# dusanerdeljan/stereo-depth

Measured on AMD Instinct MI355X. Metric: disparity maps/sec (stereo pairs/sec) at 1242x375 D=128, higher is better.
Workload: dtype f32

## Files before the change

stereo-depth_amd/csrc/k_match_fast.h:

```cpp
#pragma once
#include "smx_common.h"

namespace smx {

constexpr int FA_HALO = 11;
constexpr int FA_VALID = 64 - 2 * FA_HALO;
#ifndef SMX_FA_WAVES
#define SMX_FA_WAVES 4
#endif
constexpr int FA_WAVES = SMX_FA_WAVES;
#ifndef SMX_FA_DS_WAVES
#define SMX_FA_DS_WAVES 8
#endif
constexpr int FA_DS_WAVES = SMX_FA_DS_WAVES;
#ifndef SMX_FA_TH
#define SMX_FA_TH 24
#endif
constexpr int FA_TH = SMX_FA_TH;
#ifndef SMX_FA_TH_SMALL
#define SMX_FA_TH_SMALL 8
#endif
constexpr int FA_TH_SMALL = SMX_FA_TH_SMALL;
constexpr int FA_TH_SMALL_TALL = 12;
constexpr int FA_TH_SMALL_MID = 10;
#ifndef SMX_FA_PF
#define SMX_FA_PF 2
#endif
constexpr int FA_PF = SMX_FA_PF;
#ifndef SMX_FA_SB_PERIOD
#define SMX_FA_SB_PERIOD 2
#endif
#ifndef SMX_FA_OCC
#define SMX_FA_OCC 3
#endif
#ifndef SMX_FA_DS_OCC
#define SMX_FA_DS_OCC 4
#endif
constexpr int FA_WGCOLS = FA_VALID * FA_WAVES + 2 * FA_HALO;
#ifndef SMX_FA_WIDE_FROM
#define SMX_FA_WIDE_FROM (256 - FA_WGCOLS + 1)
#endif
constexpr int FA_WIDE_FROM = SMX_FA_WIDE_FROM;
constexpr int FA_MID_PITCH = 288;
#ifdef SMX_FA_NO_MID_PITCH
constexpr int FA_MID_UPTO = 0;
#else
constexpr int FA_MID_UPTO = FA_MID_PITCH - FA_WGCOLS + 1;
#endif
constexpr int FA_PL = (FA_VALID * FA_WAVES + 2 * FA_HALO + 7) & ~7;
constexpr int FA_BITWORDS = 64;
__host__ __device__ inline int fast_bitwords(int Dd) {
    return Dd > FA_BITWORDS * 32 ? 2 : ((Dd + 1) & ~1);
}
#define SMX_FOR_EACH_NEEDED(tbl, lo, hi, all_needed, lane, dd, rows, BODY)                                      \
    for (int g_ = (lo); g_ < (hi); g_ += 64) {                                                                  \
        const int idx_ = g_ + (lane);                                                                           \
        unsigned word_ = 0u;                                                                                    \
        if (idx_ < (hi)) word_ = (all_needed) ? ~0u : (tbl)[idx_];                                              \
        unsigned long long m_ = __ballot(word_ != 0u);                                                          \
        while (m_ != 0ull) {                                                                                    \
            const int k_ = __builtin_ctzll(m_);                                                                 \
            m_ &= m_ - 1ull;                                                                                    \
            const int dd = g_ + k_;                                                                             \
            const unsigned rows = (unsigned)__builtin_amdgcn_readlane((int)word_, k_);                          \
            BODY                                                                                                \
        }                                                                                                       \
    }

constexpr int FA_DENSE_MAX_TH = 27;
constexpr int FA_XROW = 64 + 12;
#ifndef SMX_FA_XCH_ROWS
#define SMX_FA_XCH_ROWS 2
#endif
constexpr int FA_XCH_ROWS = SMX_FA_XCH_ROWS;
constexpr int FA_XCH_FLOATS = 2 * FA_XCH_ROWS * FA_XROW;

__host__ __device__ constexpr int fast_merge_rows(int th) { return th > 8 ? (th + 1) / 2 : th; }

__host__ __device__ constexpr bool fast_prefix_exact(int th, int k_max) {
    return (long long)(th + 11) * 48195 * k_max * k_max < (1LL << 24);
}
__host__ __device__ constexpr bool fast_prefix_form(int th, int pr, bool p1only, bool dsplit, int pk16, bool argb, bool dense) {
#ifdef SMX_FA_NO_PREFIX
    return false;
#else
    if (pk16 != 2 || !fast_prefix_exact(th, 2)) return false;
    if (dsplit) return th == FA_TH_SMALL_TALL;
    (void)pr; (void)p1only; (void)argb; (void)dense;
    return true;
#endif
}

template <int PR> inline size_t fast_lds_bytes(int th, int Dd, bool dsplit = false) {
    const size_t nw = dsplit ? FA_DS_WAVES : FA_WAVES;
    return (size_t)(th + 22) * (FA_PL + PR) * sizeof(unsigned short) + nw * fast_bitwords(Dd) * sizeof(unsigned) +
           nw * FA_XCH_FLOATS * sizeof(float) + (dsplit ? nw * fast_merge_rows(th) * 64 * 2 * sizeof(float) : 0);
}

__device__ __forceinline__ float dpp_shr1(float v) {
    return __int_as_float(__builtin_amdgcn_update_dpp(0, __float_as_int(v), 0x138, 0xf, 0xf, true));
}
__device__ __forceinline__ float dpp_shl1(float v) {
    return __int_as_float(__builtin_amdgcn_update_dpp(0, __float_as_int(v), 0x130, 0xf, 0xf, true));
}
__device__ __forceinline__ unsigned dppu_sum3(unsigned v) {
    unsigned t = (unsigned)__builtin_amdgcn_update_dpp(0, (int)v, 0x138, 0xf, 0xf, true) + v;
    asm("" : "+v"(t));
    return t + (unsigned)__builtin_amdgcn_update_dpp(0, (int)v, 0x130, 0xf, 0xf, true);
}

__device__ __forceinline__ void store_u32off(float *base_uniform, unsigned off_elems, float v) {
    *(float *)((char *)base_uniform + (size_t)(off_elems * 4u)) = v;
}

__device__ __forceinline__ void atomic_or_u32off(unsigned *base_uniform, unsigned off_words, unsigned bits) {
    atomicOr((unsigned *)((char *)base_uniform + (size_t)(off_words * 4u)), bits);
}

template <int NK, int NW, bool ROUND = false>
__device__ __forceinline__ void fast_stage(unsigned short *tile, int pitch, const float *img, int h, int w,
                                           int row0, int col0, int rows, int cols, float unit, int wv, int lane) {
    int cidx[NK];
    {
        int c = wrapi(col0 + lane, w);
        const int cstep = 64 % w;
#pragma unroll
        for (int k = 0; k < NK; ++k) {
            cidx[k] = c;
            c += cstep;
            c = c >= w ? c - w : c;
        }
    }
    int ra = wrapi(row0 + wv, h);
    const int rstep = (2 * NW) % h, rhalf = NW % h;
    for (int r = wv; r < rows; r += 2 * NW) {
        const int r2 = r + NW;
        int rb = ra + rhalf;
        rb = rb >= h ? rb - h : rb;
        const float *src = img + (size_t)ra * w;
        const float *src2 = img + (size_t)(r2 < rows ? rb : ra) * w;
        float v[NK], v2[NK];
#pragma unroll
        for (int k = 0; k < NK; ++k) {
            const bool in = lane + 64 * k < cols;
            v[k] = in ? src[cidx[k]] : 0.f;
            v2[k] = in ? src2[cidx[k]] : 0.f;
        }
        unsigned short *dst = tile + r * pitch, *dst2 = tile + r2 * pitch;
#pragma unroll
        for (int k = 0; k < NK; ++k) {
            if (lane + 64 * k < cols) {
                dst[lane + 64 * k] = (unsigned short)(ROUND ? unit * v[k] + 0.5f : unit * v[k]);
                if (r2 < rows) dst2[lane + 64 * k] = (unsigned short)(ROUND ? unit * v2[k] + 0.5f : unit * v2[k]);
            }
        }
        ra += rstep;
        ra = ra >= h ? ra - h : ra;
    }
}

__host__ __device__ constexpr bool fast_units_form(int th, int pr, bool dsplit, bool argb) {
#ifdef SMX_FA_STAGE_F32
    (void)th; (void)pr; (void)dsplit; (void)argb;
    return false;
#else
    return dsplit ? th != FA_TH_SMALL_MID : (pr != 320 || argb);
#endif
}
#ifndef SMX_FA_STAGE_LOADS
#define SMX_FA_STAGE_LOADS 8
#endif
template <int NK, int NW, bool WITH_LEFT>
__device__ __forceinline__ void fast_stage_units(unsigned short *tile, int pitch, const unsigned short *img, int col0, int cols,
                                                 unsigned short *ltile, const unsigned short *limg, int lcol0, int lcols,
                                                 int h, int w, int upitch, int row0, int rows, int wv, int lane) {
    constexpr int NB = SMX_FA_STAGE_LOADS / (NK + (WITH_LEFT ? 1 : 0));
    typedef unsigned u32x2 __attribute__((ext_vector_type(2)));
    unsigned coff[NK], lcoff = 0u;
    bool in[NK], lin = false;
#pragma unroll
    for (int k = 0; k < NK; ++k) {
        in[k] = 256 * k + 4 * lane < cols;
        coff[k] = 2u * (unsigned)wrapi(col0 + 256 * k + 4 * lane, w);
    }
    if (WITH_LEFT) {
        lin = 4 * lane < lcols;
        lcoff = 2u * (unsigned)wrapi(lcol0 + 4 * lane, w);
    }
    const int wvu = __builtin_amdgcn_readfirstlane(wv);
    int ra = wrapi(row0 + wvu, h);
    const int rstep = NW % h;
    for (int r0 = wvu; r0 < rows; r0 += NB * NW) {
        u32x2 v[NB][NK], lv[NB];
#pragma unroll
        for (int j = 0; j < NB; ++j) {
            const size_t roff = (size_t)ra * upitch;
#pragma unroll
            for (int k = 0; k < NK; ++k)
                __builtin_memcpy(&v[j][k], __builtin_assume_aligned((const char *)(img + roff) + coff[k], 2), 8);
            if (WITH_LEFT) __builtin_memcpy(&lv[j], __builtin_assume_aligned((const char *)(limg + roff) + lcoff, 2), 8);
            ra += rstep;
            ra = ra >= h ? ra - h : ra;
        }
#pragma unroll
        for (int j = 0; j < NB; ++j) {
            const int r = r0 + j * NW;
            if (r < rows) {
#pragma unroll
                for (int k = 0; k < NK; ++k)
                    if (in[k]) __builtin_memcpy(__builtin_assume_aligned(tile + r * pitch + 256 * k + 4 * lane, 8), &v[j][k], 8);
                if (WITH_LEFT && lin) __builtin_memcpy(__builtin_assume_aligned(ltile + r * FA_PL + 4 * lane, 8), &lv[j], 8);
            }
        }
    }
}

struct FastLane {
    const unsigned short *lptr, *rptr;
    float *xch;
    unsigned c255;
    float inv;
    bool store_ok;
    int rows_ok;
    int colidx;
    size_t row0;
    size_t plane;
    unsigned *cand;
    unsigned cand_off_a, cand_off_b;
    unsigned long long cand_mask_a, cand_mask_b;
    unsigned cand_rstride;
    int x0;
};

typedef float f32x2 __attribute__((ext_vector_type(2)));
typedef __attribute__((address_space(3))) f32x2 fa_lds_f32x2;

__device__ __forceinline__ void argb_update(int kbyte, int &word, float m, float best, int dsel) {
    if (kbyte == 0)
        asm volatile("v_cmp_gt_f32 vcc, %1, %2\n\tv_cndmask_b32_sdwa %0, %0, %3, vcc dst_sel:BYTE_0 dst_unused:UNUSED_PRESERVE src0_sel:BYTE_0 src1_sel:BYTE_0"
                     : "+v"(word) : "v"(m), "v"(best), "v"(dsel) : "vcc");
    else if (kbyte == 1)
        asm volatile("v_cmp_gt_f32 vcc, %1, %2\n\tv_cndmask_b32_sdwa %0, %0, %3, vcc dst_sel:BYTE_1 dst_unused:UNUSED_PRESERVE src0_sel:BYTE_1 src1_sel:BYTE_0"
                     : "+v"(word) : "v"(m), "v"(best), "v"(dsel) : "vcc");
    else if (kbyte == 2)
        asm volatile("v_cmp_gt_f32 vcc, %1, %2\n\tv_cndmask_b32_sdwa %0, %0, %3, vcc dst_sel:BYTE_2 dst_unused:UNUSED_PRESERVE src0_sel:BYTE_2 src1_sel:BYTE_0"
                     : "+v"(word) : "v"(m), "v"(best), "v"(dsel) : "vcc");
    else
        asm volatile("v_cmp_gt_f32 vcc, %1, %2\n\tv_cndmask_b32_sdwa %0, %0, %3, vcc dst_sel:BYTE_3 dst_unused:UNUSED_PRESERVE src0_sel:BYTE_3 src1_sel:BYTE_0"
                     : "+v"(word) : "v"(m), "v"(best), "v"(dsel) : "vcc");
}

template <int TH, int PR, bool P1ONLY, int PK16, int MODE = 0, bool ARGB = false, bool DENSE = false, bool PREFIX = false>
__device__ __forceinline__ void fast_pass_pair(const MatchParams &p, const FastLane &ln, int d,
                                               bool valid_b, float (&best)[TH], int (&arg)[TH],
                                               const unsigned short *rptr_b_in = nullptr, int db = 0,
                                               const unsigned *argpk = nullptr, int am_a = 0, int ap_a = 0,
                                               int am_b = 0, int ap_b = 0, const unsigned *vpk = nullptr,
                                               unsigned *hits = nullptr, unsigned rowmask = ~0u,
                                               float *dmb = nullptr, float *dma = nullptr, float *dcp = nullptr,
                                               float *dfirst = nullptr) {
    static_assert(!PREFIX || (PK16 == 2 && fast_prefix_exact(TH, 2)), "prefix form: K <= 2 and every prefix below 2^24");
    constexpr int NQ = TH + 20;
    constexpr int Q9 = PREFIX ? 11 : 12, Q21 = PREFIX ? 17 : 18;
    f32x2 s1 = {0.f, 0.f}, s2 = {0.f, 0.f};
    unsigned k1 = 0u, k2 = 0u;
    const unsigned c255pk = ln.c255 * 0x10001u;
    f32x2 r3[NQ], r9[NQ], r21[NQ];
    unsigned lv[TH + 22], rva[TH + 22], rvb[TH + 22];
    f32x2 vs = {0.f, 0.f}, cs = {0.f, 0.f}, hs = {0.f, 0.f};
    f32x2 t_m3 = {0.f, 0.f}, t_p3 = {0.f, 0.f}, u_m6 = {0.f, 0.f}, u_p6 = {0.f, 0.f};
    const int lane_ = threadIdx.x & 63;
#ifdef SMX_FA_ARGMAX2
    int dva = d, dvb = d + 1;
    if (ARGB && MODE == 0) asm volatile("" : "+v"(dva), "+v"(dvb));
#endif
    const unsigned short *rptr_b = (MODE == 0 || MODE == 3) ? ln.rptr - (valid_b ? 1 : 0) : rptr_b_in;
    (void)db;
#pragma unroll
    for (int rr_ = 0; rr_ < TH + 22 + FA_PF; ++rr_) {
        if (rr_ < TH + 22) {
            lv[rr_] = ln.lptr[rr_ * FA_PL];
            rva[rr_] = ln.rptr[rr_ * PR];
            rvb[rr_] = rptr_b[rr_ * PR];
        }
        if (rr_ >= FA_PF) {
            const int r = rr_ - FA_PF;
            f32x2 s0 = {0.f, 0.f};
            unsigned k0 = 0u;
            if (PK16) {
                const unsigned sa = __builtin_amdgcn_sad_u16(lv[r], rva[r], 0u);
                const unsigned sb = __builtin_amdgcn_sad_u16(lv[r], rvb[r], 0u);
                k0 = c255pk - ((sb << 16) | sa);
            } else {
                s0.x = (float)(ln.c255 - __builtin_amdgcn_sad_u16(lv[r], rva[r], 0u));
                s0.y = (float)(ln.c255 - __builtin_amdgcn_sad_u16(lv[r], rvb[r], 0u));
            }
            if (r >= 2) {
                const int q = r - 2;
                f32x2 x3;
                if (PK16 == 2) {
                    const unsigned v3 = (k2 + k1) + k0;
                    const unsigned cv = dppu_sum3(v3);
                    const unsigned y3 = dppu_sum3(cv);
                    x3.x = (float)(y3 & 0xffffu);
                    x3.y = (float)(y3 >> 16);
                } else if (PK16 == 1) {
                    const unsigned v3 = (k2 + k1) + k0;
                    const unsigned cvp = dppu_sum3(v3);
                    f32x2 cv;
                    cv.x = (float)(cvp & 0xffffu);
                    cv.y = (float)(cvp >> 16);
                    x3.x = (dpp_shr1(cv.x) + cv.x) + dpp_shl1(cv.x);
                    x3.y = (dpp_shr1(cv.y) + cv.y) + dpp_shl1(cv.y);
                } else {
                    const f32x2 v3 = (s2 + s1) + s0;
                    f32x2 cv;
                    cv.x = (dpp_shr1(v3.x) + v3.x) + dpp_shl1(v3.x);
                    cv.y = (dpp_shr1(v3.y) + v3.y) + dpp_shl1(v3.y);
                    x3.x = (dpp_shr1(cv.x) + cv.x) + dpp_shl1(cv.x);
                    x3.y = (dpp_shr1(cv.y) + cv.y) + dpp_shl1(cv.y);
                }
                if (PREFIX && q > 0) r3[q] = r3[q > 0 ? q - 1 : 0] + x3;
                else r3[q] = x3;
                if (q >= Q9) r9[q - 6] = (t_m3 + r3[q - 6]) + t_p3;
                if (q >= Q21) r21[q - 9] = (u_m6 + u_p6) + r3[q - 9];
#ifdef SMX_EXP_NOXCH
                if (q >= Q9 - 1 && q + 1 < NQ) { t_m3 = r3[q - 5]; t_p3 = r3[q - 4]; }
                if (q >= Q21 - 1 && q + 1 < NQ) { u_m6 = r9[q - 8]; u_p6 = r9[q - 7]; }
#else
                if (q >= Q9 - 1 && q + 1 < NQ) {
                    f32x2 *x3b = (f32x2 *)ln.xch + lane_;
                    x3b[6] = r3[q - 5];
                    __builtin_amdgcn_wave_barrier();
                    {
                        const volatile fa_lds_f32x2 *xr = (const volatile fa_lds_f32x2 *)x3b;
                        t_m3 = xr[3]; t_p3 = xr[9];
                    }
                }
                if (q >= Q21 - 1 && q + 1 < NQ) {
                    f32x2 *x9b = (f32x2 *)(ln.xch + (FA_XCH_ROWS > 1 ? 2 * FA_XROW : 0)) + lane_;
                    x9b[6] = r9[q - 8];
                    __builtin_amdgcn_wave_barrier();
                    {
                        const volatile fa_lds_f32x2 *xr = (const volatile fa_lds_f32x2 *)x9b;
                        u_m6 = xr[0]; u_p6 = xr[12];
                    }
                }
#endif
                if (PREFIX) {
                    if (q >= 20) {
                        vs = q >= 21 ? r3[q] - r3[q - 21] : r3[q];
                        cs = r9[q - 6] - r9[q - 15];
                        hs = r21[q - 9] - r21[q - 12];
                    }
                } else {
                    vs += r3[q];
                    if (q >= 21) vs -= r3[q - 21];
                    if (q >= 12) cs += r9[q - 6];
                    if (q >= 21) cs -= r9[q - 15];
                    if (q >= 18) hs += r21[q - 9];
                    if (q >= 21) hs -= r21[q - 12];
                }
                if (q >= 20) {
                    const int o = q - 20;
                    const f32x2 agg = (hs * vs) * cs;
                    if ((MODE == 1 || MODE == 2) && !((rowmask >> o) & 1u)) {
                    } else if (MODE == 2) {
                        unsigned upk_w = argpk[o >> 1], vpk_w = vpk[o >> 1];
                        asm volatile("" : "+v"(upk_w), "+v"(vpk_w));
                        const unsigned U = (upk_w >> (16 * (o & 1))) & 0xffffu;
                        const unsigned V = (vpk_w >> (16 * (o & 1))) & 0xffffu;
                        int ci = ln.colidx;
                        asm volatile("" : "+v"(ci));
                        const unsigned off = (unsigned)(o * p.w + ci);
                        float *cp = p.costs + ln.row0;
                        auto put = [&](unsigned dl1, unsigned o2, float v) {
                            const size_t pl = dl1 == 1u ? 0 : (dl1 == 2u ? 1 : 2);
                            cp[pl * ln.plane + o2] = v * ln.inv;
                        };
                        const unsigned a1 = (unsigned)(d + 1) - U, a2 = V + 1u - (unsigned)d, a3 = (unsigned)(am_a + 1) - U;
                        const unsigned b1 = (unsigned)(db + 1) - U, b2 = V + 1u - (unsigned)db;
                        if (a1 < 3u) put(a1, off, agg.x);
                        if (a2 < 3u) put(a2, off + 1u, agg.x);
                        if (a3 < 3u) put(a3, off, agg.x);
                        if (b1 < 3u) put(b1, off, agg.y);
                        if (b2 < 3u) put(b2, off + 1u, agg.y);
                    } else if (MODE == 4) {
                        best[o] = __builtin_fmaxf(__builtin_fmaxf(best[o], agg.x), agg.y);
                    } else if (MODE == 3) {
                        const bool okp = ln.store_ok && o < ln.rows_ok;
                        const unsigned long long ma = __ballot(okp && agg.x >= best[o]);
                        const unsigned long long mb = __ballot(okp && agg.y >= best[o]);
                        const unsigned tr = (unsigned)(((ln.x0 + o) >> 4) - (ln.x0 >> 4));
                        const unsigned h4 = ((ma & ln.cand_mask_a) != 0ull ? 1u : 0u) | ((ma & ln.cand_mask_b) != 0ull ? 2u : 0u) |
                                            ((mb & ln.cand_mask_a) != 0ull ? 4u : 0u) | ((mb & ln.cand_mask_b) != 0ull ? 8u : 0u);
                        *hits |= h4 << (4u * tr);
                    } else if (MODE == 1) {
                        const int a = (int)((argpk[o >> 1] >> (16 * (o & 1))) & 0xffffu);
                        int ci = ln.colidx;
                        asm volatile("" : "+v"(ci));
                        const unsigned off = (unsigned)(o * p.w + ci);
                        const bool xa = a == am_a, xb = a == ap_a;
                        if (xa || a == am_b) store_u32off(p.costs + ln.row0 + ln.plane, off, (xa ? agg.x : agg.y) * ln.inv);
                        if (xb || a == ap_b) store_u32off(p.costs + ln.row0 + 2 * ln.plane, off, (xb ? agg.x : agg.y) * ln.inv);
                    } else {
                        if constexpr (DENSE) {
                            const float after_d = valid_b ? agg.y : __builtin_nanf("");
                            dma[o] = (dma[o] != dma[o]) ? agg.x : dma[o];
                            const bool ca = (agg.x > best[o]) | (d == 0);
                            const float b1 = __builtin_fmaxf(best[o], agg.x);
                            dmb[o] = ca ? dcp[o] : dmb[o];
                            dma[o] = ca ? after_d : dma[o];
                            const bool cb = agg.y > b1;
                            dmb[o] = cb ? agg.x : dmb[o];
                            dma[o] = cb ? __builtin_nanf("") : dma[o];
                            dcp[o] = agg.y;
                            if (dfirst) dfirst[o] = agg.x;
                        }
#if !defined(SMX_FA_ARGMAX2)
                        const float m = __builtin_fmaxf(__builtin_fmaxf(best[o], agg.x), agg.y);
                        const int dsel = (agg.x == m) ? d : d + 1;
#ifndef SMX_EXP_NOARG
                        if (ARGB) {
                            argb_update(o & 3, arg[o >> 2], m, best[o], dsel);
                        } else {
                            const bool changed = m > best[o];
                            arg[o] = changed ? dsel : arg[o];
                        }
#else
                        (void)dsel;
#endif
                        best[o] = m;
#else
                        if (ARGB) {
                            argb_update(o & 3, arg[o >> 2], agg.x, best[o], dva);
                            best[o] = __builtin_fmaxf(best[o], agg.x);
                            argb_update(o & 3, arg[o >> 2], agg.y, best[o], dvb);
                            best[o] = __builtin_fmaxf(best[o], agg.y);
                        } else {
                            const float m = __builtin_fmaxf(__builtin_fmaxf(best[o], agg.x), agg.y);
                            const int dsel = (agg.x == m) ? d : d + 1;
                            arg[o] = m > best[o] ? dsel : arg[o];
                            best[o] = m;
                        }
#endif
                    }
                }
            }
            s2 = s1;
            s1 = s0;
            k2 = k1;
            k1 = k0;
        }
        if ((rr_ % SMX_FA_SB_PERIOD) == SMX_FA_SB_PERIOD - 1)
            __builtin_amdgcn_sched_barrier(0);
    }
}

constexpr int FA_STAT_WG_STRIDE_DS = 16;
template <bool DSPLIT>
__device__ __forceinline__ void fast_stats_report(const MatchParams &p, int b, int wg_lin, int wv, int marches, bool window) {
    if (!p.fast_stats || b % p.fast_stride != 0) return;
    if (DSPLIT && wg_lin % FA_STAT_WG_STRIDE_DS != 0) return;
    const bool win = window && (!DSPLIT || wv == 0);
    const unsigned long long v = ((unsigned long long)(unsigned)marches << 24) | (win ? 1ull : 0ull);
    if (v != 0ull) (void)__hip_atomic_fetch_add(p.fast_stats, v, __ATOMIC_RELAXED, __HIP_MEMORY_SCOPE_AGENT);
}

template <int TU, int NH, int PR, int PK16, bool PREFIX, class StageRight>
__device__ __forceinline__ void fast_stacked_tail(const MatchParams &p, const BlockIdx3 &blk, const FastLane &ln, const float (&best)[TU * NH],
                                                  const int (&argb)[TU * NH], const unsigned short *Rt, unsigned *bits, int wcol, int x0,
                                                  bool active, StageRight &&stage_right) {
    constexpr int ND = PR - FA_WGCOLS + 1;
    const int lane = threadIdx.x & 63, wv = threadIdx.x >> 6;
    const int h = p.h, w = p.w, Dd = p.Dd, BW = fast_bitwords(Dd);
    const bool all_needed = Dd > FA_BITWORDS * 32;
    unsigned *wbits = bits + wv * BW;
#pragma unroll
    for (int hh = 0; hh < NH; ++hh) {
        float bh[TU];
        int ah[TU];
#pragma unroll
        for (int o = 0; o < TU; ++o) {
            bh[o] = best[hh * TU + o];
            ah[o] = (argb[(hh * TU + o) >> 2] >> (8 * ((hh * TU + o) & 3))) & 0xff;
        }
        FastLane lh = ln;
        lh.lptr = ln.lptr + hh * TU * FA_PL;
        lh.row0 = ln.row0 + (size_t)(hh * TU) * w;
        lh.rows_ok = max(0, min(TU, h - x0 - hh * TU));
        const unsigned short *Rh = Rt + hh * TU * PR;
        unsigned dup_left = 0u;
#ifndef SMX_FA_NO_DEDUP
        if (!all_needed) {
#pragma unroll
            for (int o = 0; o < TU; ++o) {
                const int la = __builtin_amdgcn_update_dpp(-1, ah[o], 0x138, 0xf, 0xf, false);
                dup_left |= (la == ah[o] ? 1u : 0u) << o;
            }
            const int left_ok = __builtin_amdgcn_update_dpp(0, lh.store_ok ? 1 : 0, 0x138, 0xf, 0xf, false);
            if (!left_ok) dup_left = 0u;
        }
#endif
        if (lh.store_ok) {
#pragma unroll
            for (int o = 0; o < TU; ++o) {
                if (o < lh.rows_ok) {
                    const unsigned off = (unsigned)(o * w + lh.colidx);
                    store_u32off(p.wta + lh.row0, off, (float)ah[o] + (float)p.dmin);
                    const bool nv = !(bh[o] > SMX_FLT_MIN);
                    store_u32off(p.costs + lh.row0, off, nv ? 0.0f : bh[o] * lh.inv);
                    if (!all_needed && !((dup_left >> o) & 1u)) {
                        const int dn = (ah[o] + 1 == Dd) ? 0 : ah[o] + 1;
                        const int dp = (ah[o] == 0) ? Dd - 1 : ah[o] - 1;
                        atomicOr(&wbits[dn], 1u << o);
                        atomicOr(&wbits[dp], 1u << o);
                    }
                }
            }
        }
        int marches2 = 0;
        unsigned argpk[(TU + 1) / 2];
#pragma unroll
        for (int o = 0; o < (TU + 1) / 2; ++o) argpk[o] = 0u;
#pragma unroll
        for (int o = 0; o < TU; ++o)
            argpk[o >> 1] |= ((lh.store_ok && o < lh.rows_ok) ? (unsigned)ah[o] : 0xffffu) << (16 * (o & 1));
        for (int d0 = 0; d0 < Dd; d0 += ND) {
            const int nd = min(ND, Dd - d0);
            if (Dd > ND) stage_right(d0, nd);
            else __syncthreads();
            if (active) {
                auto march = [&](int dda, int ddb, unsigned rows) {
                    const int da = d0 + dda, db = d0 + ddb;
                    ++marches2;
                    lh.rptr = Rh + wcol + lane + (nd - 1 - dda);
                    fast_pass_pair<TU, PR, false, PK16, 1, false, false, PREFIX>(p, lh, da, false, bh, ah, Rh + wcol + lane + (nd - 1 - ddb), db, argpk,
                                                           da == 0 ? Dd - 1 : da - 1, da + 1 == Dd ? 0 : da + 1,
                                                           db == 0 ? Dd - 1 : db - 1, db + 1 == Dd ? 0 : db + 1, nullptr, nullptr, rows);
                };
                int pend = -1;
                unsigned pend_rows = 0u;
                SMX_FOR_EACH_NEEDED(wbits + d0, 0, nd, all_needed, lane, dd, rows, {
                    if (pend < 0) { pend = dd; pend_rows = rows; }
                    else { march(pend, dd, pend_rows | rows); pend = -1; }
                })
                if (pend >= 0) march(pend, pend, pend_rows);
            }
        }
        if (lane == 0) fast_stats_report<false>(p, blk.z, (int)(blk.x + gridDim.x * blk.y), wv, marches2, active && lh.rows_ok > 0);
        if (hh + 1 < NH)
            for (int e = lane; e < BW; e += 64) wbits[e] = 0u;
    }
}

template <int TH, int PR, bool P1ONLY, bool DSPLIT, int PK16, bool ARGB = false, bool DENSE = false>
__device__ __forceinline__ void match_fast_body(const MatchParams &p, const BlockIdx3 &blk) {
    static_assert(!DENSE || !P1ONLY, "the dense form is a pass 1 with neighbours: min_disparity = 0");
    static_assert(!DENSE || !DSPLIT || !ARGB, "latency shape: one register per winner");
    constexpr int NW = DSPLIT ? FA_DS_WAVES : FA_WAVES;
    constexpr int WGCOLS = DSPLIT ? 64 : FA_WGCOLS;
    constexpr int ND = PR - WGCOLS + 1;
    constexpr int NH = TH > 32 ? 2 : 1;
    constexpr int TU = TH / NH;
    constexpr bool PREFIX = fast_prefix_form(TH, PR, P1ONLY, DSPLIT, PK16, ARGB, DENSE);
    static_assert(NH == 1 || (TH == 2 * TU && TU <= 32 && ARGB && !DSPLIT && !DENSE && !P1ONLY),
                  "stacked bands: two unit bands, byte-packed winners, throughput shape, sparse form");
    const int b = blk.z;

    extern __shared__ __attribute__((aligned(16))) unsigned short fsmem[];
    unsigned short *Lt = fsmem;
    unsigned short *Rt = fsmem + (TH + 22) * FA_PL;
    unsigned *bits = (unsigned *)(Rt + (TH + 22) * PR);
    const int BW = fast_bitwords(p.Dd);

    const int tid = threadIdx.x;
    const int lane = tid & 63;
    const int wv = tid >> 6;
    const int h = p.h, w = p.w, Dd = p.Dd;
    const int cwg0 = blk.x * (DSPLIT ? 1 : FA_WAVES) * FA_VALID;
    const int cw0 = cwg0 + (DSPLIT ? 0 : wv * FA_VALID);
    const int wcol = DSPLIT ? 0 : wv * FA_VALID;
    const bool active = cw0 < w;
    const int x0 = blk.y * TH;
    const int col = cw0 - FA_HALO + lane;
    constexpr bool UNITS = fast_units_form(TH, PR, DSPLIT, ARGB);
    const float *Lp = p.Ld + (size_t)b * h * w;
    const float *Rp = p.Rd + (size_t)b * h * w;
    const unsigned short *Lup = p.Lu + (size_t)b * h * p.upitch;
    const unsigned short *Rup = p.Ru + (size_t)b * h * p.upitch;
    const float unit = p.unit;

    FastLane ln;
    ln.xch = (float *)(bits + NW * BW) + wv * FA_XCH_FLOATS;
    ln.c255 = (unsigned)(255.0f * unit);
    ln.inv = 1.0f / (unit * unit * unit);
    ln.store_ok = active && lane >= FA_HALO && lane < FA_HALO + FA_VALID && col < w;
    ln.rows_ok = min(TH, h - x0);
    ln.plane = (size_t)p.B * h * w;
    ln.row0 = ((size_t)b * h + x0) * w;
    ln.colidx = ln.store_ok ? col : 0;
    ln.lptr = Lt + wcol + lane;

    float best[TH];
    int arg[TH];
#pragma unroll
    for (int o = 0; o < TH; ++o) { best[o] = SMX_FLT_MIN; arg[o] = 0; }
    float dmb[DENSE ? TH : 1], dma[DENSE ? TH : 1], dcp[DENSE ? TH : 1];
    float dfirst[DENSE && DSPLIT ? TH : 1];
#pragma unroll
    for (int o = 0; o < (DENSE ? TH : 1); ++o) { dmb[o] = 0.f; dma[o] = 0.f; dcp[o] = 0.f; }
#pragma unroll
    for (int o = 0; o < (DENSE && DSPLIT ? TH : 1); ++o) dfirst[o] = 0.f;

    if constexpr (!UNITS)
        fast_stage<(WGCOLS + 63) / 64, NW>(Lt, FA_PL, Lp, h, w, x0 - FA_HALO, cwg0 - FA_HALO, TH + 22, WGCOLS, unit, wv, lane);
    for (int e = tid; e < NW * BW; e += 64 * NW) bits[e] = 0u;

    auto stage_right = [&](int d0, int nd, bool with_left = false) {
        __syncthreads();
        const int cbase = cwg0 - FA_HALO - (p.dmin + d0 + nd - 1);
        if constexpr (!UNITS)
            fast_stage<(PR + 63) / 64, NW>(Rt, PR, Rp, h, w, x0 - FA_HALO, cbase, TH + 22, WGCOLS + nd - 1, unit, wv, lane);
        else if (with_left)
            fast_stage_units<(PR + 255) / 256, NW, true>(Rt, PR, Rup, cbase, WGCOLS + nd - 1, Lt, Lup, cwg0 - FA_HALO, WGCOLS, h, w, p.upitch,
                                                         x0 - FA_HALO, TH + 22, wv, lane);
        else
            fast_stage_units<(PR + 255) / 256, NW, false>(Rt, PR, Rup, cbase, WGCOLS + nd - 1, nullptr, nullptr, 0, 0, h, w, p.upitch,
                                                          x0 - FA_HALO, TH + 22, wv, lane);
        __syncthreads();
    };

    if constexpr (UNITS) stage_right(0, min(ND, Dd), true);
    for (int d0 = 0; d0 < Dd; d0 += ND) {
        const int nd = min(ND, Dd - d0);
        if (!UNITS || d0 > 0) stage_right(d0, nd);
        if (active) {
            const int q4 = ((nd + 2 * NW - 1) / (2 * NW)) * 2;
            const int dd_lo = DSPLIT ? min(nd, wv * q4) : 0;
            const int dd_hi = DSPLIT ? min(nd, dd_lo + q4) : nd;
            for (int dd = dd_lo; dd < dd_hi; dd += 2) {
                ln.rptr = Rt + wcol + lane + (nd - 1 - dd);
                if constexpr (DENSE)
                    fast_pass_pair<TH, PR, P1ONLY, PK16, 0, ARGB, true, PREFIX>(p, ln, d0 + dd, dd + 1 < dd_hi, best, arg, nullptr, 0, nullptr,
                                                                         0, 0, 0, 0, nullptr, nullptr, ~0u, dmb, dma, dcp,
                                                                         DSPLIT && dd == dd_lo ? dfirst : nullptr);
                else
                    fast_pass_pair<TH, PR, P1ONLY, PK16, 0, ARGB, false, PREFIX>(p, ln, d0 + dd, dd + 1 < dd_hi, best, arg);
            }
        }
    }
    if constexpr (NH > 1) {
        fast_stacked_tail<TU, NH, PR, PK16, PREFIX>(p, blk, ln, best, arg, Rt, bits, wcol, x0, active, stage_right);
        return;
    }
    if (ARGB) {
        int packed[(TH + 3) / 4];
#pragma unroll
        for (int o = 0; o < (TH + 3) / 4; ++o) packed[o] = arg[o];
#pragma unroll
        for (int o = 0; o < TH; ++o) arg[o] = (packed[o >> 2] >> (8 * (o & 3))) & 0xff;
    }
    float *mrg = (float *)(bits + NW * BW) + NW * FA_XCH_FLOATS;
    if constexpr (DSPLIT && DENSE) {
        constexpr int MR = fast_merge_rows(TH), R2 = (NW * MR * 2) / (NW * 6);
        static_assert(R2 >= 1 && R2 <= NW, "merge buffer: at least one row of six values per wave");
        const int q4 = ((Dd + 2 * NW - 1) / (2 * NW)) * 2;
        const int nk = (Dd + q4 - 1) / q4;
#pragma unroll 1
        for (int o0 = 0; o0 < TH; o0 += R2) {
            __syncthreads();
#pragma unroll
            for (int o = 0; o < TH; ++o) {
                if (o >= o0 && o < o0 + R2) {
                    float *q = mrg + ((size_t)(wv * R2 + (o - o0)) * 64 + lane) * 6;
                    q[0] = best[o]; q[1] = __int_as_float(arg[o]); q[2] = dmb[o]; q[3] = dma[o]; q[4] = dfirst[o]; q[5] = dcp[o];
                }
            }
            __syncthreads();
            const int j = wv;
            if (j < R2 && o0 + j < ln.rows_ok && ln.store_ok) {
                auto M = [&](int k, int f) { return mrg[((size_t)(k * R2 + j) * 64 + lane) * 6 + f]; };
                float bb = SMX_FLT_MIN;
                int aa = 0, kw = 0;
                for (int k = 0; k < nk; ++k) {
                    const float bk = M(k, 0);
                    const bool g = bk > bb;
                    aa = g ? __float_as_int(M(k, 1)) : aa;
                    kw = g ? k : kw;
                    bb = g ? bk : bb;
                }
                float mb = M(kw, 2), ma = M(kw, 3);
                if (aa == kw * q4) mb = M(kw > 0 ? kw - 1 : nk - 1, 5);
                if (ma != ma) ma = M(kw + 1 < nk ? kw + 1 : 0, 4);
                const unsigned off = (unsigned)((o0 + j) * w + ln.colidx);
                store_u32off(p.wta + ln.row0, off, (float)aa + (float)p.dmin);
                store_u32off(p.costs + ln.row0, off, !(bb > SMX_FLT_MIN) ? 0.0f : bb * ln.inv);
                store_u32off(p.costs + ln.row0 + ln.plane, off, ma * ln.inv);
                store_u32off(p.costs + ln.row0 + 2 * ln.plane, off, mb * ln.inv);
            }
        }
        return;
    }
    if (DSPLIT) {
        constexpr int MR = fast_merge_rows(TH);
#pragma unroll
        for (int o0 = 0; o0 < TH; o0 += MR) {
            __syncthreads();
#pragma unroll
            for (int o = o0; o < o0 + MR && o < TH; ++o) {
                mrg[((wv * MR + (o - o0)) * 64 + lane) * 2] = best[o];
                mrg[((wv * MR + (o - o0)) * 64 + lane) * 2 + 1] = __int_as_float(arg[o]);
            }
            __syncthreads();
#pragma unroll
            for (int o = o0; o < o0 + MR && o < TH; ++o) {
                float bb = SMX_FLT_MIN;
                int aa = 0;
#pragma unroll
                for (int k = 0; k < NW; ++k) {
                    const float bk = mrg[((k * MR + (o - o0)) * 64 + lane) * 2];
                    const int ak = __float_as_int(mrg[((k * MR + (o - o0)) * 64 + lane) * 2 + 1]);
                    const bool g = bk > bb;
                    aa = g ? ak : aa;
                    bb = g ? bk : bb;
                }
                best[o] = bb;
                arg[o] = aa;
            }
        }
    }

    const bool all_needed = Dd > FA_BITWORDS * 32;
    unsigned dup_left = 0u;
#ifndef SMX_FA_NO_DEDUP
    if (!DENSE && !P1ONLY && !all_needed) {
#pragma unroll
        for (int o = 0; o < TH; ++o) {
            const int la = __builtin_amdgcn_update_dpp(-1, arg[o], 0x138, 0xf, 0xf, false);
            dup_left |= (la == arg[o] ? 1u : 0u) << o;
        }
        const int left_ok = __builtin_amdgcn_update_dpp(0, ln.store_ok ? 1 : 0, 0x138, 0xf, 0xf, false);
        if (!left_ok) dup_left = 0u;
    }
#endif
    if (ln.store_ok) {
        unsigned *wbits = bits + (DSPLIT ? 0 : wv) * BW;
#pragma unroll
        for (int o = 0; o < TH; ++o) {
            if (o < ln.rows_ok && (!DSPLIT || o % NW == wv)) {
                const unsigned off = (unsigned)(o * w + ln.colidx);
                store_u32off(p.wta + ln.row0, off, (float)arg[o] + (float)p.dmin);
                const bool nv = !(best[o] > SMX_FLT_MIN);
                store_u32off(p.costs + ln.row0, off, nv ? 0.0f : best[o] * ln.inv);
                if constexpr (DENSE) {
                    store_u32off(p.costs + ln.row0 + 2 * ln.plane, off, (arg[o] == 0 ? dcp[o] : dmb[o]) * ln.inv);
                    if (dma[o] != dma[o]) {
                        if (!all_needed) atomicOr(&wbits[0], 1u << o);
                    } else {
                        store_u32off(p.costs + ln.row0 + ln.plane, off, dma[o] * ln.inv);
                    }
                } else
                if (!P1ONLY && !all_needed && !((dup_left >> o) & 1u)) {
                    const int dn = (arg[o] + 1 == Dd) ? 0 : arg[o] + 1;
                    const int dp = (arg[o] == 0) ? Dd - 1 : arg[o] - 1;
                    atomicOr(&wbits[dn], 1u << o);
                    atomicOr(&wbits[dp], 1u << o);
                }
            }
        }
    }
    if (P1ONLY) return;

    int marches2 = 0;
    unsigned argpk[(TH + 1) / 2];
#pragma unroll
    for (int o = 0; o < (TH + 1) / 2; ++o) argpk[o] = 0u;
#pragma unroll
    for (int o = 0; o < TH; ++o)
        argpk[o >> 1] |= ((ln.store_ok && o < ln.rows_ok) ? (unsigned)arg[o] : 0xffffu) << (16 * (o & 1));
    for (int d0 = 0; d0 < (DENSE ? 1 : Dd); d0 += ND) {
        const int nd = min(ND, Dd - d0);
        if (Dd > ND) stage_right(d0, nd);
        else __syncthreads();
        if (active) {
            const unsigned *mybits = bits + (DSPLIT ? 0 : wv) * BW;
            const int q4 = ((nd + 2 * NW - 1) / (2 * NW)) * 2;
            const int dd_lo = DSPLIT ? min(nd, wv * q4) : 0;
            const int dd_hi = DSPLIT ? min(nd, dd_lo + q4) : nd;
            auto march = [&](int dda, int ddb, unsigned rows) {
                const int da = d0 + dda, db = d0 + ddb;
                ++marches2;
                ln.rptr = Rt + wcol + lane + (nd - 1 - dda);
                fast_pass_pair<TH, PR, false, PK16, 1, false, false, PREFIX>(p, ln, da, false, best, arg, Rt + wcol + lane + (nd - 1 - ddb), db, argpk,
                                                       da == 0 ? Dd - 1 : da - 1, da + 1 == Dd ? 0 : da + 1,
                                                       db == 0 ? Dd - 1 : db - 1, db + 1 == Dd ? 0 : db + 1, nullptr, nullptr, rows);
            };
            int pend = -1;
            unsigned pend_rows = 0u;
#ifndef SMX_EXP_NOPASS2
            if constexpr (DSPLIT) {
                (void)dd_lo; (void)dd_hi;
                int seen = 0;
                SMX_FOR_EACH_NEEDED(mybits + d0, 0, nd, all_needed, lane, dd, rows, {
                    const bool mine = (seen >> 1) % NW == wv;
                    ++seen;
                    if (mine) {
                        if (pend < 0) { pend = dd; pend_rows = rows; }
                        else { march(pend, dd, pend_rows | rows); pend = -1; }
                    }
                })
            } else {
                SMX_FOR_EACH_NEEDED(mybits + d0, dd_lo, dd_hi, all_needed, lane, dd, rows, {
                    if (pend < 0) { pend = dd; pend_rows = rows; }
                    else { march(pend, dd, pend_rows | rows); pend = -1; }
                })
// ... 165 lines not shown
```

Before: 102,800.

## Schedule stacked-band tail passes jointly with per-band tables and mixed full/half passes

The stacked-unit tail used to process the two unit bands separately. It now keeps a separate needed-disparity bitmap for each band and walks both bitmaps together. Disparities needed by both bands are paired into full-height passes; those needed by only one band are paired into half-height passes, and leftovers are packed by a small state machine. To make room for the second table, the second exchange row of LDS is given up, and a rowmask_hi parameter supports row masks over 32 rows. This is meant to cut redundant or poorly paired refinement passes, at the cost of more control flow and one fewer exchange buffer.

```diff
diff --git a/stereo-depth_amd/csrc/k_match_fast.h b/stereo-depth_amd/csrc/k_match_fast.h
--- a/stereo-depth_amd/csrc/k_match_fast.h
+++ b/stereo-depth_amd/csrc/k_match_fast.h
@@ -90,6 +90,16 @@
     return true;
 #endif
 }
+
+__host__ __device__ constexpr int fast_tables(int th) {
+#ifdef SMX_FA_STACK_TAIL_HALVES
+    (void)th;
+    return 1;
+#else
+    return th > 32 ? 2 : 1;
+#endif
+}
+__host__ __device__ constexpr int fast_xch_rows(int th) { return fast_tables(th) > 1 ? 1 : FA_XCH_ROWS; }
 
 template <int PR> inline size_t fast_lds_bytes(int th, int Dd, bool dsplit = false) {
     const size_t nw = dsplit ? FA_DS_WAVES : FA_WAVES;
@@ -250,7 +260,7 @@
                      : "+v"(word) : "v"(m), "v"(best), "v"(dsel) : "vcc");
 }
 
-template <int TH, int PR, bool P1ONLY, int PK16, int MODE = 0, bool ARGB = false, bool DENSE = false, bool PREFIX = false>
+template <int TH, int PR, bool P1ONLY, int PK16, int MODE = 0, bool ARGB = false, bool DENSE = false, bool PREFIX = false, int XR = FA_XCH_ROWS>
 __device__ __forceinline__ void fast_pass_pair(const MatchParams &p, const FastLane &ln, int d,
                                                bool valid_b, float (&best)[TH], int (&arg)[TH],
                                                const unsigned short *rptr_b_in = nullptr, int db = 0,
@@ -258,7 +268,7 @@
                                                int am_b = 0, int ap_b = 0, const unsigned *vpk = nullptr,
                                                unsigned *hits = nullptr, unsigned rowmask = ~0u,
                                                float *dmb = nullptr, float *dma = nullptr, float *dcp = nullptr,
-                                               float *dfirst = nullptr) {
+                                               float *dfirst = nullptr, unsigned rowmask_hi = 0u) {
     static_assert(!PREFIX || (PK16 == 2 && fast_prefix_exact(TH, 2)), "prefix form: K <= 2 and every prefix below 2^24");
     constexpr int NQ = TH + 20;
     constexpr int Q9 = PREFIX ? 11 : 12, Q21 = PREFIX ? 17 : 18;
@@ -338,7 +348,7 @@
                     }
                 }
                 if (q >= Q21 - 1 && q + 1 < NQ) {
-                    f32x2 *x9b = (f32x2 *)(ln.xch + (FA_XCH_ROWS > 1 ? 2 * FA_XROW : 0)) + lane_;
+                    f32x2 *x9b = (f32x2 *)(ln.xch + (XR > 1 ? 2 * FA_XROW : 0)) + lane_;
                     x9b[6] = r9[q - 8];
                     __builtin_amdgcn_wave_barrier();
                     {
@@ -364,7 +374,7 @@
                 if (q >= 20) {
                     const int o = q - 20;
                     const f32x2 agg = (hs * vs) * cs;
-                    if ((MODE == 1 || MODE == 2) && !((rowmask >> o) & 1u)) {
+                    if ((MODE == 1 || MODE == 2) && !(((o < 32 ? rowmask : rowmask_hi) >> (o & 31)) & 1u)) {
                     } else if (MODE == 2) {
                         unsigned upk_w = argpk[o >> 1], vpk_w = vpk[o >> 1];
                         asm volatile("" : "+v"(upk_w), "+v"(vpk_w));
@@ -468,9 +478,9 @@
 }
 
 template <int TU, int NH, int PR, int PK16, bool PREFIX, class StageRight>
-__device__ __forceinline__ void fast_stacked_tail(const MatchParams &p, const BlockIdx3 &blk, const FastLane &ln, const float (&best)[TU * NH],
-                                                  const int (&argb)[TU * NH], const unsigned short *Rt, unsigned *bits, int wcol, int x0,
-                                                  bool active, StageRight &&stage_right) {
+__device__ __forceinline__ void fast_stacked_tail_halves(const MatchParams &p, const BlockIdx3 &blk, const FastLane &ln, const float (&best)[TU * NH],
+                                                         const int (&argb)[TU * NH], const unsigned short *Rt, unsigned *bits, int wcol, int x0,
+                                                         bool active, StageRight &&stage_right) {
     constexpr int ND = PR - FA_WGCOLS + 1;
     const int lane = threadIdx.x & 63, wv = threadIdx.x >> 6;
     const int h = p.h, w = p.w, Dd = p.Dd, BW = fast_bitwords(Dd);
@@ -554,6 +564,199 @@
     }
 }
 
+enum FastTailLeftover { FT_NONE = 0, FT_FULL_BB, FT_FULL_BU, FT_FULL_BL, FT_FULL_UL, FT_HALVES, FT_UPPER, FT_LOWER };
+__host__ __device__ constexpr int fast_tail_leftover(bool both, bool upper, bool lower) {
+    return both ? (upper ? (lower ? FT_HALVES : FT_FULL_BU) : (lower ? FT_FULL_BL : FT_FULL_BB))
+                : (upper ? (lower ? FT_FULL_UL : FT_UPPER) : (lower ? FT_LOWER : FT_NONE));
+}
+__host__ __device__ constexpr int fast_tail_leftover_rows(int code, int tu) {
+    return code == FT_NONE ? 0 : (code == FT_UPPER || code == FT_LOWER ? tu + 22 : (code == FT_HALVES ? 2 * (tu + 22) : 2 * tu + 22));
+}
+__host__ __device__ constexpr long fast_tail_rows(int nb, int nu, int nl, int tu) {
+    return (long)(nb / 2) * (2 * tu + 22) + (long)(nu / 2 + nl / 2) * (tu + 22) +
+           fast_tail_leftover_rows(fast_tail_leftover(nb & 1, nu & 1, nl & 1), tu);
+}
+__host__ __device__ constexpr long fast_tail_rows_halves(int nb, int nu, int nl, int tu) {
+    return (long)((nb + nu + 1) / 2 + (nb + nl + 1) / 2) * (tu + 22);
+}
+
+template <int TU, int NH, int PR, int PK16, bool PREFIX>
+__device__ __forceinline__ void fast_stacked_tail(const MatchParams &p, const BlockIdx3 &blk, const FastLane &ln, const float (&best)[TU * NH],
+                                                  const int (&argb)[TU * NH], const unsigned short *Rt, unsigned *bits, int wcol, int x0,
+                                                  bool active) {
+    static_assert(NH == 2 && TU % 2 == 0 && TU < 32 && fast_tables(TU * NH) == NH, "two unit bands, a table each; argpk holds two rows a word");
+    static_assert(PR == 256 && FA_WIDE_FROM <= PR - FA_WGCOLS + 1, "stacked bands: a single right-tile chunk");
+    constexpr int TH = TU * NH, XR = fast_xch_rows(TH);
+    const int lane = threadIdx.x & 63, wv = threadIdx.x >> 6;
+    const int h = p.h, w = p.w, Dd = p.Dd, nd = p.Dd, BW = fast_bitwords(Dd);
+    const bool all_needed = Dd > FA_BITWORDS * 32;
+    unsigned *wbits = bits + wv * NH * BW;
+    unsigned argpk[TH / 2];
+#pragma unroll
+    for (int hh = 0; hh < NH; ++hh) {
+        float bh[TU];
+        int ah[TU];
+#pragma unroll
+        for (int o = 0; o < TU; ++o) {
+            bh[o] = best[hh * TU + o];
+            ah[o] = (argb[(hh * TU + o) >> 2] >> (8 * ((hh * TU + o) & 3))) & 0xff;
+        }
+        FastLane lh = ln;
+        lh.row0 = ln.row0 + (size_t)(hh * TU) * w;
+        lh.rows_ok = max(0, min(TU, h - x0 - hh * TU));
+        unsigned *hbits = wbits + hh * BW;
+        unsigned dup_left = 0u;
+#ifndef SMX_FA_NO_DEDUP
+        if (!all_needed) {
+#pragma unroll
+            for (int o = 0; o < TU; ++o) {
+                const int la = __builtin_amdgcn_update_dpp(-1, ah[o], 0x138, 0xf, 0xf, false);
+                dup_left |= (la == ah[o] ? 1u : 0u) << o;
+            }
+            const int left_ok = __builtin_amdgcn_update_dpp(0, lh.store_ok ? 1 : 0, 0x138, 0xf, 0xf, false);
+            if (!left_ok) dup_left = 0u;
+        }
+#endif
+        if (lh.store_ok) {
+#pragma unroll
+            for (int o = 0; o < TU; ++o) {
+                if (o < lh.rows_ok) {
+                    const unsigned off = (unsigned)(o * w + lh.colidx);
+                    store_u32off(p.wta + lh.row0, off, (float)ah[o] + (float)p.dmin);
+                    const bool nv = !(bh[o] > SMX_FLT_MIN);
+                    store_u32off(p.costs + lh.row0, off, nv ? 0.0f : bh[o] * lh.inv);
+                    if (!all_needed && !((dup_left >> o) & 1u)) {
+                        const int dn = (ah[o] + 1 == Dd) ? 0 : ah[o] + 1;
+                        const int dp = (ah[o] == 0) ? Dd - 1 : ah[o] - 1;
+                        atomicOr(&hbits[dn], 1u << o);
+                        atomicOr(&hbits[dp], 1u << o);
+                    }
+                }
+            }
+        }
+#pragma unroll
+        for (int o = 0; o < TU / 2; ++o) argpk[hh * (TU / 2) + o] = 0u;
+#pragma unroll
+        for (int o = 0; o < TU; ++o)
+            argpk[hh * (TU / 2) + (o >> 1)] |= ((lh.store_ok && o < lh.rows_ok) ? (unsigned)ah[o] : 0xffffu) << (16 * (o & 1));
+    }
+#ifdef SMX_FA_STACK_TAIL_BARRIER
+    __syncthreads();
+#endif
+    __builtin_amdgcn_wave_barrier();
+    if (p.fast_stats && active) {
+#pragma unroll
+        for (int hh = 0; hh < NH; ++hh) {
+            int n = 0;
+            for (int g0 = 0; g0 < nd; g0 += 64) {
+                const bool in = g0 + lane < nd;
+                n += __builtin_popcountll(__ballot(in && (all_needed || wbits[hh * BW + g0 + lane] != 0u)));
+            }
+            if (lane == 0) fast_stats_report<false>(p, blk.z, (int)(blk.x + gridDim.x * blk.y), wv, (n + 1) / 2, h - x0 - hh * TU > 0);
+        }
+    }
+    {
+        if (active) {
+            enum { K_NONE, K_FULL, K_UPPER, K_LOWER };
+            const unsigned *tbl_u = wbits, *tbl_l = wbits + BW;
+            enum { P_B, P_U, P_L, R_BU, R_BL, R_U, R_L };
+            int pst[7] = {-1, -1, -1, 0, 0, 0, 0};
+            auto pget = [&](int i) { return pst[i]; };
+            auto pset = [&](int i, int v) { pst[i] = v; };
+            int g = -64;
+            unsigned word_u = 0u, word_l = 0u;
+            unsigned long long m = 0ull;
+            for (;;) {
+                int kind = K_NONE, dda = 0, ddb = 0;
+                unsigned r_u = 0u, r_l = 0u;
+                const int pb = pget(P_B);
+                if (pb == -2) {
+                    kind = K_LOWER; dda = pget(P_U); ddb = pget(P_L); r_u = (unsigned)pget(R_L);
+                    pset(P_B, -1); pset(P_U, -1); pset(P_L, -1);
+                } else if (m != 0ull) {
+                    const int k = __builtin_ctzll(m);
+                    m &= m - 1ull;
+                    const int dd = g + k;
+                    const unsigned ru = (unsigned)__builtin_amdgcn_readlane((int)word_u, k);
+                    const unsigned rl = (unsigned)__builtin_amdgcn_readlane((int)word_l, k);
+                    if (ru != 0u && rl != 0u) {
+                        if (pb < 0) { pset(P_B, dd); pset(R_BU, (int)ru); pset(R_BL, (int)rl); }
+                        else { kind = K_FULL; dda = pb; ddb = dd; r_u = (unsigned)pget(R_BU) | ru; r_l = (unsigned)pget(R_BL) | rl; pset(P_B, -1); }
+                    } else if (ru != 0u) {
+                        const int pu = pget(P_U);
+                        if (pu < 0) { pset(P_U, dd); pset(R_U, (int)ru); }
+                        else { kind = K_UPPER; dda = pu; ddb = dd; r_u = (unsigned)pget(R_U) | ru; pset(P_U, -1); }
+                    } else {
+                        const int pl = pget(P_L);
+                        if (pl < 0) { pset(P_L, dd); pset(R_L, (int)rl); }
+                        else { kind = K_LOWER; dda = pl; ddb = dd; r_u = (unsigned)pget(R_L) | rl; pset(P_L, -1); }
+                    }
+                } else if (g + 64 < nd) {
+                    g += 64;
+                    const int idx = g + lane;
+                    word_u = 0u;
+                    word_l = 0u;
+                    if (idx < nd) {
+                        word_u = all_needed ? ~0u : tbl_u[idx];
+                        word_l = all_needed ? ~0u : tbl_l[idx];
+                    }
+                    m = __ballot((word_u | word_l) != 0u);
+                } else {
+                    const int pu = pget(P_U), pl = pget(P_L);
+                    const int code = fast_tail_leftover(pb >= 0, pu >= 0, pl >= 0);
+                    if (code == FT_NONE) break;
+                    const unsigned pb_u = (unsigned)pget(R_BU), pb_l = (unsigned)pget(R_BL), pu_r = (unsigned)pget(R_U), pl_r = (unsigned)pget(R_L);
+                    if (code == FT_FULL_BB) { kind = K_FULL; dda = pb; ddb = pb; r_u = pb_u; r_l = pb_l; }
+                    else if (code == FT_FULL_BU) { kind = K_FULL; dda = pb; ddb = pu; r_u = pb_u | pu_r; r_l = pb_l; }
+                    else if (code == FT_FULL_BL) { kind = K_FULL; dda = pb; ddb = pl; r_u = pb_u; r_l = pb_l | pl_r; }
+                    else if (code == FT_FULL_UL) { kind = K_FULL; dda = pu; ddb = pl; r_u = pu_r; r_l = pl_r; }
+                    else if (code == FT_UPPER) { kind = K_UPPER; dda = pu; ddb = pu; r_u = pu_r; }
+                    else if (code == FT_LOWER) { kind = K_LOWER; dda = pl; ddb = pl; r_u = pl_r; }
+                    if (code == FT_HALVES) {
+                        kind = K_UPPER; dda = pb; ddb = pu; r_u = pb_u | pu_r;
+                        pset(R_L, (int)(pl_r | pb_l)); pset(P_U, pb); pset(P_B, -2);
+                    } else {
+                        pset(P_B, -1); pset(P_U, -1); pset(P_L, -1);
+                    }
+                }
+                if (kind == K_NONE) continue;
+                const int da = dda, db = ddb;
+                const int am_a = da == 0 ? Dd - 1 : da - 1, ap_a = da + 1 == Dd ? 0 : da + 1;
+                const int am_b = db == 0 ? Dd - 1 : db - 1, ap_b = db + 1 == Dd ? 0 : db + 1;
+                if (kind == K_FULL) {
+                    float bd[TH];
+                    int ad[TH];
+#pragma unroll
+                    for (int o = 0; o < TH; ++o) { bd[o] = 0.f; ad[o] = 0; }
+                    FastLane lf = ln;
+                    lf.rptr = Rt + wcol + lane + (nd - 1 - dda);
+                    fast_pass_pair<TH, PR, false, PK16, 1, false, false, PREFIX, XR>(p, lf, da, false, bd, ad, Rt + wcol + lane + (nd - 1 - ddb), db, argpk,
+                                                                                 am_a, ap_a, am_b, ap_b, nullptr, nullptr, r_u | (r_l << TU), nullptr,
+                                                                                 nullptr, nullptr, nullptr, r_l >> (32 - TU));
+                } else {
+                    float bd[TU];
+                    int ad[TU];
+#pragma unroll
+                    for (int o = 0; o < TU; ++o) { bd[o] = 0.f; ad[o] = 0; }
+                    FastLane lh = ln;
+                    if (kind == K_UPPER) {
+                        lh.rptr = Rt + wcol + lane + (nd - 1 - dda);
+                        fast_pass_pair<TU, PR, false, PK16, 1, false, false, PREFIX, XR>(p, lh, da, false, bd, ad, Rt + wcol + lane + (nd - 1 - ddb), db, argpk,
+                                                                                     am_a, ap_a, am_b, ap_b, nullptr, nullptr, r_u);
+                    } else {
+                        const unsigned short *Rh = Rt + TU * PR;
+                        lh.lptr = ln.lptr + TU * FA_PL;
+                        lh.row0 = ln.row0 + (size_t)TU * w;
+                        lh.rptr = Rh + wcol + lane + (nd - 1 - dda);
+                        fast_pass_pair<TU, PR, false, PK16, 1, false, false, PREFIX, XR>(p, lh, da, false, bd, ad, Rh + wcol + lane + (nd - 1 - ddb), db,
+                                                                                     argpk + TU / 2, am_a, ap_a, am_b, ap_b, nullptr, nullptr, r_u);
+                    }
+                }
+            }
+        }
+    }
+}
+
 template <int TH, int PR, bool P1ONLY, bool DSPLIT, int PK16, bool ARGB = false, bool DENSE = false>
 __device__ __forceinline__ void match_fast_body(const MatchParams &p, const BlockIdx3 &blk) {
     static_assert(!DENSE || !P1ONLY, "the dense form is a pass 1 with neighbours: min_disparity = 0");
@@ -572,6 +775,10 @@
     unsigned short *Lt = fsmem;
     unsigned short *Rt = fsmem + (TH + 22) * FA_PL;
     unsigned *bits = (unsigned *)(Rt + (TH + 22) * PR);
+    constexpr int NT = fast_tables(TH);
+    constexpr int XR = fast_xch_rows(TH);
+    static_assert(NT == 1 || (XR == 1 && FA_XCH_ROWS == 2 && (NT - 1) * ((ND + 1) & ~1) <= 2 * FA_XROW),
+                  "the second table fits the exchange row it replaces: fast_lds_bytes is unchanged");
     const int BW = fast_bitwords(p.Dd);
 
     const int tid = threadIdx.x;
@@ -592,7 +799,7 @@
     const float unit = p.unit;
 
     FastLane ln;
-    ln.xch = (float *)(bits + NW * BW) + wv * FA_XCH_FLOATS;
+    ln.xch = (float *)(bits + NW * NT * BW) + wv * (2 * XR * FA_XROW);
     ln.c255 = (unsigned)(255.0f * unit);
     ln.inv = 1.0f / (unit * unit * unit);
     ln.store_ok = active && lane >= FA_HALO && lane < FA_HALO + FA_VALID && col < w;
@@ -615,7 +822,7 @@
 
     if constexpr (!UNITS)
         fast_stage<(WGCOLS + 63) / 64, NW>(Lt, FA_PL, Lp, h, w, x0 - FA_HALO, cwg0 - FA_HALO, TH + 22, WGCOLS, unit, wv, lane);
-    for (int e = tid; e < NW * BW; e += 64 * NW) bits[e] = 0u;
+    for (int e = tid; e < NW * NT * BW; e += 64 * NW) bits[e] = 0u;
 
     auto stage_right = [&](int d0, int nd, bool with_left = false) {
         __syncthreads();
@@ -642,16 +849,20 @@
             for (int dd = dd_lo; dd < dd_hi; dd += 2) {
                 ln.rptr = Rt + wcol + lane + (nd - 1 - dd);
                 if constexpr (DENSE)
-                    fast_pass_pair<TH, PR, P1ONLY, PK16, 0, ARGB, true, PREFIX>(p, ln, d0 + dd, dd + 1 < dd_hi, best, arg, nullptr, 0, nullptr,
+                    fast_pass_pair<TH, PR, P1ONLY, PK16, 0, ARGB, true, PREFIX, XR>(p, ln, d0 + dd, dd + 1 < dd_hi, best, arg, nullptr, 0, nullptr,
                                                                          0, 0, 0, 0, nullptr, nullptr, ~0u, dmb, dma, dcp,
                                                                          DSPLIT && dd == dd_lo ? dfirst : nullptr);
                 else
-                    fast_pass_pair<TH, PR, P1ONLY, PK16, 0, ARGB, false, PREFIX>(p, ln, d0 + dd, dd + 1 < dd_hi, best, arg);
+                    fast_pass_pair<TH, PR, P1ONLY, PK16, 0, ARGB, false, PREFIX, XR>(p, ln, d0 + dd, dd + 1 < dd_hi, best, arg);
             }
         }
     }
     if constexpr (NH > 1) {
-        fast_stacked_tail<TU, NH, PR, PK16, PREFIX>(p, blk, ln, best, arg, Rt, bits, wcol, x0, active, stage_right);
+#ifdef SMX_FA_STACK_TAIL_HALVES
+        fast_stacked_tail_halves<TU, NH, PR, PK16, PREFIX>(p, blk, ln, best, arg, Rt, bits, wcol, x0, active, stage_right);
+#else
+        fast_stacked_tail<TU, NH, PR, PK16, PREFIX>(p, blk, ln, best, arg, Rt, bits, wcol, x0, active);
+#endif
         return;
     }
     if (ARGB) {
@@ -661,7 +872,7 @@
 #pragma unroll
         for (int o = 0; o < TH; ++o) arg[o] = (packed[o >> 2] >> (8 * (o & 3))) & 0xff;
     }
-    float *mrg = (float *)(bits + NW * BW) + NW * FA_XCH_FLOATS;
+    float *mrg = (float *)(bits + NW * NT * BW) + NW * FA_XCH_FLOATS;
     if constexpr (DSPLIT && DENSE) {
         constexpr int MR = fast_merge_rows(TH), R2 = (NW * MR * 2) / (NW * 6);
         static_assert(R2 >= 1 && R2 <= NW, "merge buffer: at least one row of six values per wave");
```

Measured after the change: 104,200, median of 6. 1.01x the previous value.
